# yalue/cudabrot

Measured on AMD Instinct MI355X. Metric: Msamples/sec (escaping points) + HBM GB/s, 4096x4096 max_iter=20000, 1/2/4/8 GPU, higher is better.
Workload: dtype f64

## Files before the change

### cudabrot_amd/capi.py

```python

import ctypes as C
import os

import numpy as np

CB_DEFAULT_THREADS = 512 * 512
CB_SAMPLES_PER_THREAD = 50
CB_DEFAULT_RNG_SEED = 1337
CB_KERNEL_DEFAULT = 0
CB_KERNEL_SIMPLE = 1
CB_KERNEL_TIMED = 2
CB_KERNEL_FULL_ITERATE = 3
CB_TONE_AUTO, CB_TONE_LUT, CB_TONE_THRESHOLDS = 0, 1, 2
CB_KERNEL_FLAG_BURNING_SHIP = 0x100
CB_KERNEL_FLAG_DRAIN = 0x200
CB_KERNEL_FLAG_ANTI = 0x400
CB_POWER_MIN, CB_POWER_MAX = 3, 8
CB_KERNEL_POWER_MASK = 0xF000


def CB_KERNEL_POWER(degree):
    degree = int(degree)
    if not CB_POWER_MIN <= degree <= CB_POWER_MAX:
        raise ValueError("degree must be an integer from %d to %d" % (CB_POWER_MIN, CB_POWER_MAX))
# ... 82 lines not shown
            "cycles_replay",
            "cycles_total",
            "rt_not_first_start",
            "rt_last_end",
            "rt_wave_life_sum",
        )
    ]

    def as_dict(self):
        return {n: int(getattr(self, n)) for n, _ in self._fields_}


class ScatterArray(C.Structure):

    _fields_ = [("offset", C.c_uint64), ("bytes", C.c_uint64)]


SCATTER_ARRAYS = ("wave_count stream a_count a_base grouped region_start region_count region_group owner_first "
                  "group_first group_regions n_regions chunk_desc chunk_list run_start slice_base sorted").split()


class ScatterLayout(C.Structure):

    _fields_ = [
        (n, C.c_uint32)
        for n in ("enabled n_waves cap n_tiles tiles_x tiles_y n_planes two_level n_groups chunked chunks_per_wave "
                  "max_regions e_row_shift e_col_mask e_row_mask e_chan_shift e_chan_mask reserved").split()
    ] + [(n, ScatterArray) for n in SCATTER_ARRAYS]

    def arrays(self):
        return {n: (int(getattr(self, n).offset), int(getattr(self, n).bytes))
                for n in SCATTER_ARRAYS if getattr(self, n).bytes}


def _share_torch_hip_runtime():
    if os.environ.get("CUDABROT_AMD_SYSTEM_HIP") == "1":
        return None
    try:
        import importlib.util

        spec = importlib.util.find_spec("torch")
    except (ImportError, ValueError):
        spec = None
    if spec is None or not spec.submodule_search_locations:
        return None
    cand = os.path.join(list(spec.submodule_search_locations)[0], "lib", "libamdhip64.so")
    if not os.path.exists(cand):
        return None
    C.CDLL(cand, mode=C.RTLD_GLOBAL)
    return cand


def _load():
    path = library_path()
    if not os.path.exists(path):
        raise ImportError(
            "cudabrot_amd: %s is missing -- build it with `make` (or __graft_entry__.build()); "
            "there is no CPU fallback" % path
        )
    _share_torch_hip_runtime()
    lib_ = C.CDLL(path)
    vp, u32, u64, i32 = C.c_void_p, C.c_uint32, C.c_uint64, C.c_int
    dims_p, it_p, cnt_p = C.POINTER(FractalDimensions), C.POINTER(IterationControl), C.POINTER(Counters)
    col_p = C.POINTER(ColorParams)
    sigs = {
        "cb_abi_version": (i32, []),
        "cb_error_string": (C.c_char_p, [i32]),
        "cb_debug_knob": (C.c_char_p, [C.c_char_p]),
        "cb_debug_last_draw_kernel": (i32, []),
        "cb_debug_interior_map_level": (i32, []),
        "cb_renderer_interior_map_level": (i32, [vp]),
        "cb_recompute_pixel_deltas": (i32, [dims_p, C.POINTER(C.c_char_p)]),
        "cb_rng_state_bytes": (C.c_size_t, [u32]),
        "cb_initialize_rng": (i32, [u64, u64, u32, vp, vp]),
        "cb_scatter_workspace_bytes": (C.c_size_t, [dims_p, u32, u32]),
        "cb_scatter_workspace_bytes_channels": (C.c_size_t, [dims_p, i32, u32, u32]),
        "cb_draw_buddhabrot": (i32, [dims_p, vp, it_p, vp, u32, u32, vp, i32, vp, C.c_size_t, vp, vp]),
        "cb_carry_bytes": (C.c_size_t, [u32]),
        "cb_draw_buddhabrot_channels": (i32, [dims_p, vp, it_p, i32, vp, u32, u32, vp, i32, vp, C.c_size_t, vp, vp]),
        "cb_flush_scatter_channels": (i32, [dims_p, vp, i32, u32, vp, C.c_size_t, vp]),
        "cb_renderer_finish": (i32, [vp]),
        "cb_flush_scatter": (i32, [dims_p, vp, u32, vp, C.c_size_t, vp]),
        "cb_debug_scatter_layout": (i32, [dims_p, i32, u32, vp, C.c_size_t, C.POINTER(ScatterLayout)]),
        "cb_renderer_create": (i32, [C.POINTER(vp), i32, dims_p, it_p, u64, u64, u32]),
        "cb_renderer_create_channels": (i32, [C.POINTER(vp), i32, dims_p, it_p, i32, u64, u64, u32]),
        "cb_renderer_grayscale_plane": (i32, [vp, i32, C.c_double, i32, vp, C.POINTER(u64), C.POINTER(C.c_double)]),
        "cb_renderer_render_passes": (i32, [vp, u32, i32]),
        "cb_renderer_prepare": (i32, [vp, i32]),
        "cb_renderer_read_histogram": (i32, [vp, vp]),
        "cb_renderer_write_histogram": (i32, [vp, vp]),
        "cb_renderer_read_counters": (i32, [vp, cnt_p]),
        "cb_renderer_read_rng_states": (i32, [vp, vp]),
        "cb_renderer_write_rng_states": (i32, [vp, vp]),
        "cb_renderer_device_histogram": (vp, [vp]),
        "cb_renderers_reduce": (i32, [C.POINTER(vp), i32]),
        "cb_renderer_destroy": (None, [vp]),
        "cb_set_grayscale_pixels": (None, [vp, i32, i32, C.c_double, vp, C.POINTER(u64), C.POINTER(C.c_double)]),
        "cb_save_image": (i32, [C.c_char_p, vp, i32, i32]),
        "cb_save_image_be": (i32, [C.c_char_p, vp, i32, i32]),
        "cb_tone_value": (C.c_uint16, [u64, u64, C.c_double]),
        "cb_tone_map_device": (i32, [vp, i32, i32, C.c_double, i32, vp, C.POINTER(u64), C.POINTER(C.c_double), vp]),
        "cb_renderer_grayscale_image": (i32, [vp, C.c_double, i32, vp, C.POINTER(u64), C.POINTER(C.c_double)]),
        "cb_compose_color": (i32, [C.POINTER(vp), i32, i32, col_p, vp, vp]),
        "cb_compose_color_device": (i32, [C.POINTER(vp), i32, i32, C.c_double, i32, col_p, vp, vp, vp]),
        "cb_renderer_color_image": (i32, [vp, C.POINTER(i32), C.c_double, i32, col_p, vp, vp]),
        "cb_save_ppm_be": (i32, [C.c_char_p, vp, i32, i32]),
        "cb_focus_mask_bytes": (C.c_size_t, [i32]),
        "cb_focus_probe": (i32, [dims_p, it_p, vp, u32, u32, i32, vp, vp, i32, vp]),
        "cb_focus_cells": (i32, [i32, vp, i32, vp, C.POINTER(u32)]),
        "cb_draw_buddhabrot_focus": (i32, [dims_p, vp, it_p, vp, u32, u32, vp, i32, i32, vp, u32, vp]),
        "cb_renderer_set_focus": (i32, [vp, i32, u32, i32, i32]),
        "cb_renderer_focus_cells": (i32, [vp, C.POINTER(u32), C.POINTER(u32)]),
        "cb_draw_buddhabrot_projected": (i32, [dims_p, vp, it_p, C.POINTER(C.c_double), vp, u32, u32, vp, i32, vp]),
        "cb_renderer_set_projection": (i32, [vp, C.POINTER(C.c_double)]),
        "cb_renderer_projection": (i32, [vp, C.POINTER(C.c_double)]),
    }
    for name, (res, args) in sigs.items():
        fn = getattr(lib_, name)
        fn.restype = res
        fn.argtypes = args
    return lib_


lib = _load()
EXPORTED_SYMBOLS = (
    "cb_abi_version cb_error_string cb_debug_knob cb_debug_last_draw_kernel cb_debug_interior_map_level cb_renderer_interior_map_level cb_recompute_pixel_deltas cb_rng_state_bytes cb_initialize_rng "
    "cb_scatter_workspace_bytes cb_scatter_workspace_bytes_channels cb_carry_bytes cb_draw_buddhabrot cb_flush_scatter cb_renderer_create "
    "cb_renderer_render_passes cb_renderer_finish "
    "cb_renderer_read_histogram "
    "cb_renderer_write_histogram cb_renderer_read_counters cb_renderer_device_histogram "
    "cb_renderer_destroy cb_set_grayscale_pixels cb_save_image cb_save_image_be cb_tone_value "
    "cb_tone_map_device cb_renderer_grayscale_image cb_renderer_read_rng_states cb_renderer_write_rng_states "
    "cb_draw_buddhabrot_channels cb_flush_scatter_channels cb_renderer_create_channels cb_renderer_grayscale_plane cb_renderers_reduce "
    "cb_renderer_prepare cb_compose_color cb_compose_color_device cb_renderer_color_image cb_save_ppm_be "
    "cb_focus_mask_bytes cb_focus_probe cb_focus_cells cb_draw_buddhabrot_focus cb_renderer_set_focus cb_renderer_focus_cells "
    "cb_draw_buddhabrot_projected cb_renderer_set_projection cb_renderer_projection cb_debug_scatter_layout"
).split()


def _error_string(code):
    return lib.cb_error_string(int(code)).decode()


def _check(code, what):
    if code != 0:
        raise CudabrotError(code, what)


def recompute_pixel_deltas(dims):
    msg = C.c_char_p()
    ok = lib.cb_recompute_pixel_deltas(C.byref(dims), C.byref(msg))
    return bool(ok), (None if ok else msg.value.decode())


def rng_state_bytes(n_threads):
    return int(lib.cb_rng_state_bytes(n_threads))


def initialize_rng(seed, first_subsequence, n_threads, d_states, stream=0):
    _check(lib.cb_initialize_rng(seed, first_subsequence, n_threads, d_states, stream), "cb_initialize_rng")


def scatter_workspace_bytes(dims, n_threads, samples_per_thread, n_channels=1):
    return int(lib.cb_scatter_workspace_bytes_channels(C.byref(dims), n_channels, n_threads, samples_per_thread))


def carry_bytes(n_threads):
    return int(lib.cb_carry_bytes(n_threads))


def draw_buddhabrot(dims, d_hist, iterations, d_states, n_threads, samples_per_thread, d_counters=0,
                    kernel_variant=CB_KERNEL_DEFAULT, stream=0, d_workspace=0, workspace_bytes=0, d_carry=0):
    _check(
        lib.cb_draw_buddhabrot(C.byref(dims), d_hist, C.byref(iterations), d_states, n_threads,
                               samples_per_thread, d_counters, kernel_variant, d_workspace, workspace_bytes,
                               d_carry, stream),
        "cb_draw_buddhabrot",
    )


def flush_scatter(dims, d_hist, n_threads, d_workspace, workspace_bytes, stream=0):
    _check(lib.cb_flush_scatter(C.byref(dims), d_hist, n_threads, d_workspace, workspace_bytes, stream),
           "cb_flush_scatter")


def debug_scatter_layout(dims, n_threads, d_workspace, workspace_bytes, n_channels=0):
    out = ScatterLayout()
    _check(lib.cb_debug_scatter_layout(C.byref(dims), n_channels, n_threads, d_workspace, workspace_bytes,
                                       C.byref(out)), "cb_debug_scatter_layout")
    return out


def focus_mask_bytes(level):
    return int(lib.cb_focus_mask_bytes(int(level)))


def focus_probe(dims, iterations, d_states, n_threads, samples_per_thread, level, d_mask, d_counters=0,
                kernel_variant=CB_KERNEL_DEFAULT, stream=0):
    _check(
        lib.cb_focus_probe(C.byref(dims), C.byref(iterations), d_states, n_threads, samples_per_thread, int(level),
                           d_mask, d_counters, kernel_variant, stream),
        "cb_focus_probe",
    )


def focus_cells(level, mask, dilate=1):
    m = np.ascontiguousarray(mask, dtype=np.uint32).reshape(-1)
    if m.size * 4 != focus_mask_bytes(level):
        raise ValueError("mask size does not match the level")
    n = C.c_uint32()
    _check(lib.cb_focus_cells(int(level), m.ctypes.data, int(dilate), None, C.byref(n)), "cb_focus_cells")
    cells = np.empty(int(n.value), dtype=np.uint32)
    _check(lib.cb_focus_cells(int(level), m.ctypes.data, int(dilate), cells.ctypes.data, C.byref(n)), "cb_focus_cells")
    return cells


def draw_buddhabrot_focus(dims, d_hist, iterations, d_states, n_threads, samples_per_thread, d_counters=0,
                          kernel_variant=CB_KERNEL_DEFAULT, level=0, d_cells=0, n_cells=0, stream=0):
    _check(
# ... 237 lines not shown
```

### cudabrot_amd/csrc/scatter.hip

```cpp
#include <stdlib.h>
#include <string.h>

#include <type_traits>

#include "kernels.h"

namespace cb {

namespace {

constexpr int kSortPrioIo = 3;
constexpr int kSortPrioRank = 0;
constexpr int kGatherPrio = 0;
constexpr uint32_t kLeanBatch = 4;

constexpr uint32_t kScatterThreads = 512;
constexpr uint32_t kChunkEntries = 8192;
constexpr uint32_t kPerThread = kChunkEntries / kScatterThreads;
constexpr uint32_t kAccThreadsWide = 1024;
constexpr uint32_t kGroupShift = 10;
static_assert((1u << kGroupShift) == kGroupTiles, "group = tile >> kGroupShift");
constexpr uint32_t kReplicas = kGroupReplicas;
constexpr uint32_t kMaxGroups = 256;
constexpr uint32_t kMaxKeys = kMaxGroups * kGroupTiles;
// ... 93 lines not shown
  const uint32_t n_owners = owner_count(b);
  const uint32_t per = (n_owners + 1023u) / 1024u;
  const uint32_t o0 = threadIdx.x * per;
  if (threadIdx.x == 0) all_entries = 0ull;
  __syncthreads();
  uint32_t mine = 0;
  unsigned long long my_entries = 0;
  for (uint32_t k = 0; k < per; ++k) {
    if (o0 + k < n_owners) {
      unsigned long long begin, entries;
      uint32_t piece;
      owner_extent(b, o0 + k, &begin, &entries, &piece);
      mine += (uint32_t) ((entries + piece - 1u) / piece);
      my_entries += entries;
    }
  }
  if (my_entries) __hip_atomic_fetch_add(&all_entries, my_entries, __ATOMIC_RELAXED, __HIP_MEMORY_SCOPE_WORKGROUP);
  uint32_t total = 0;
  uint32_t r = block_exclusive_scan(mine, wave_totals, &total);
  if (threadIdx.x == 0) {
    *reinterpret_cast<unsigned long long *>(b.n_regions + 2) = b.chunked ? all_entries * kChunkWords : all_entries;
  }
  for (uint32_t k = 0; k < per; ++k) {
    const uint32_t o = o0 + k;
    if (o >= n_owners) break;
    unsigned long long begin, entries;
    uint32_t piece;
    owner_extent(b, o, &begin, &entries, &piece);
    const uint32_t regions = (uint32_t) ((entries + piece - 1u) / piece);
    b.owner_first[o] = r;
    if (b.two_level) {
      b.group_first[o] = r;
      b.group_regions[o] = regions;
    }
    r += regions;
  }
  if (threadIdx.x == 0) {
    b.owner_first[n_owners] = total;
    *b.n_regions = total;
    if (!b.two_level) {
      b.group_first[0] = 0u;
      b.group_regions[0] = total;
    }
  }
}

__global__ void __launch_bounds__(256) bin_fill_regions_kernel(BinLayout b) {
  const uint32_t r = blockIdx.x * blockDim.x + threadIdx.x;
  if (r >= *b.n_regions) return;
  uint32_t lo = 0, hi = owner_count(b);
  while (hi - lo > 1u) {
    const uint32_t mid = (lo + hi) >> 1;
    if (b.owner_first[mid] <= r) {
      lo = mid;
    } else {
      hi = mid;
    }
  }
  unsigned long long begin, entries;
  uint32_t piece;
  owner_extent(b, lo, &begin, &entries, &piece);
  const unsigned long long offset = (unsigned long long) (r - b.owner_first[lo]) * piece;
  b.region_start[r] = begin + offset;
  b.region_count[r] = (uint32_t) ((entries - offset) < piece ? (entries - offset) : piece);
  b.region_group[r] = b.two_level ? lo : 0u;
}

constexpr uint32_t kSliceTargetGroups = 12288;
constexpr uint32_t kSliceTargetGroupsTwoLevel = 6144;
static_assert(kSliceTargetGroupsTwoLevel <= kSliceTargetGroups, "the grid of the gather is sized by the larger one");
constexpr uint32_t kSliceRegionsMin = 512;
constexpr uint32_t kSliceEntriesMin = 32768;
__device__ __forceinline__ uint32_t slice_regions_for(const BinLayout &b, unsigned long long pairs,
                                                      unsigned long long entries) {
  const unsigned long long target = b.two_level ? kSliceTargetGroupsTwoLevel : kSliceTargetGroups;
  unsigned long long s = (pairs + target - 1u) / target;
  if (s < kSliceRegionsMin) s = kSliceRegionsMin;
  const unsigned long long by_entries = entries ? (kSliceEntriesMin * pairs + entries - 1u) / entries : b.slice_regions;
  if (s < by_entries) s = by_entries;
  if (s > b.slice_regions) s = b.slice_regions;
  return (uint32_t) s;
}

__global__ void __launch_bounds__(1024) bin_slice_table_kernel(BinLayout b) {
  __shared__ uint32_t wave_totals[16];
  const uint32_t nk = b.n_tiles;
  const uint32_t per = (nk + 1023u) / 1024u;
  const uint32_t t0 = threadIdx.x * per;
  unsigned long long pairs = 0;
  for (uint32_t g = 0; g < b.n_groups; ++g) {
    const uint32_t tiles = (nk - (g << kGroupShift)) < kGroupTiles ? (nk - (g << kGroupShift)) : kGroupTiles;
    pairs += (unsigned long long) tiles * b.group_regions[g];
  }
  const uint32_t S = slice_regions_for(b, pairs, *reinterpret_cast<const unsigned long long *>(b.n_regions + 2));
  if (threadIdx.x == 0) b.n_regions[1] = S;
  auto slices_of = [&](uint32_t t) { return (b.group_regions[t >> kGroupShift] + S - 1u) / S; };
  uint32_t mine = 0;
  for (uint32_t k = 0; k < per; ++k) {
    if (t0 + k < nk) mine += slices_of(t0 + k);
  }
  uint32_t total = 0;
  uint32_t run = block_exclusive_scan(mine, wave_totals, &total);
  for (uint32_t k = 0; k < per; ++k) {
    const uint32_t t = t0 + k;
    if (t < nk) {
      b.slice_base[t] = run;
      run += slices_of(t);
    }
  }
  if (threadIdx.x == 0) b.slice_base[nk] = total;
}

constexpr uint32_t kDummyPlace = kRegionEntries + 8u;
template <bool kFewTiles>
struct SortLds {
  static constexpr uint32_t kReplicas = kFewTiles ? 8u : 2u;
  static constexpr uint32_t kStride = (kFewTiles ? 256u : kGroupTiles) + 16u;
  static constexpr size_t kBytes =
      (kReplicas * kStride + 16 + 2 * kRegionChunks + 4) * sizeof(uint32_t) + (kRegionEntries + 16) * sizeof(uint16_t);
};
constexpr uint32_t kFewTilesMax = 256;
constexpr uint32_t kSortGrid = 32768;
constexpr uint32_t kRunBatch = 8;

template <bool kPlain>
__device__ __forceinline__ uint32_t sort_word(uint32_t e, uint32_t k0, const BinLayout &b) {
  if (kPlain) {
    const uint32_t key = __umul24(e >> (16 + kTileShift), b.tiles_x) + ((e & 0xffffu) >> kTileShift) - k0;
    return (key << 16) | ((e >> (16 - kTileShift)) & ((kTileSize - 1u) << kTileShift)) | (e & (kTileSize - 1u));
  }
  return ((tile_of(e, b) - k0) << 16) | offset_of(e, b);
}

template <bool kPlain, bool kFewTiles, bool kChunked = false, bool kLean = false>
__global__ void __launch_bounds__(kSortThreads, 8) bin_region_sort_kernel(BinLayout b, uint32_t skip_lean) {
  constexpr uint32_t kCntReplicas = SortLds<kFewTiles>::kReplicas, kCntStride = SortLds<kFewTiles>::kStride;
  constexpr uint32_t kDummyKey = kCntStride - 16u;
  __builtin_amdgcn_s_setprio(kSortPrioIo);
  extern __shared__ uint32_t lds[];
  uint32_t *cnt = lds + (threadIdx.x % kCntReplicas) * kCntStride;
  uint32_t *wave_totals = lds + kCntReplicas * kCntStride;
  uint2 *chunks = reinterpret_cast<uint2 *>(lds + kCntReplicas * kCntStride + 16);
  uint16_t *image = reinterpret_cast<uint16_t *>(lds + kCntReplicas * kCntStride + 16 + 2 * kRegionChunks + 4);

  const uint32_t n_regions = *b.n_regions;
  constexpr uint32_t kBatchRegions = kLean ? kRunBatch : 1u;
  for (uint32_t r_batch = blockIdx.x * kBatchRegions; r_batch < n_regions; r_batch += gridDim.x * kBatchRegions) {
  uint32_t runs[4] = {0u, 0u, 0u, 0u};
  const auto push_run = [&](uint32_t v) {
    runs[0] = __builtin_amdgcn_alignbit(runs[1], runs[0], 16);
    runs[1] = __builtin_amdgcn_alignbit(runs[2], runs[1], 16);
    runs[2] = __builtin_amdgcn_alignbit(runs[3], runs[2], 16);
    runs[3] = __builtin_amdgcn_alignbit(v, runs[3], 16);
  };
#pragma unroll 1
  for (uint32_t r = r_batch; r < r_batch + kBatchRegions; ++r) {
  if (kLean && r >= n_regions) {
    push_run(0u);
    continue;
  }
  uint32_t n = kChunked ? 0u : b.region_count[r];
  const unsigned long long start = kChunked ? (unsigned long long) r * kRegionEntries : b.region_start[r];
  const uint32_t *src = kChunked ? b.stream : (b.two_level ? b.grouped : b.stream) + start;
  const uint32_t k0 = b.region_group[r] << kGroupShift;
  const uint32_t nk = (b.n_tiles - k0) < kGroupTiles ? (b.n_tiles - k0) : kGroupTiles;
  __syncthreads();
  for (uint32_t t = threadIdx.x; t < kCntReplicas * kCntStride; t += kSortThreads) lds[t] = 0u;
  if (kChunked && threadIdx.x < 64u) {
    const uint32_t n_chunks = b.region_count[r];
    const uint2 c = threadIdx.x < n_chunks && threadIdx.x < kRegionChunks ? b.chunk_list[b.region_start[r] + threadIdx.x]
                                                                          : make_uint2(0u, 0u);
    if (threadIdx.x < kRegionChunks) chunks[threadIdx.x] = c;
    uint32_t words = c.y;
#pragma unroll
    for (uint32_t d = 32; d >= 1; d >>= 1) words += __shfl_xor(words, d, 64);
    if (threadIdx.x == 0) chunks[kRegionChunks].x = words;
  }
  __syncthreads();
  if (kChunked) n = chunks[kRegionChunks].x;

  const bool lean_region = kPlain && n != 0u && (kChunked || (start & 7ull) == 0ull);
  if (!kLean && skip_lean != 0u && lean_region) continue;
  if (kLean && !lean_region) {
    push_run(0u);
    continue;
  }
  if constexpr (kLean) {
    typedef __attribute__((address_space(3))) uint32_t *LdsWord;
    typedef __attribute__((address_space(3))) uint16_t *LdsHalf;
    const uint32_t lds0 = (uint32_t) reinterpret_cast<uintptr_t>(static_cast<void *>(lds));
    const uint32_t cnt_at = lds0 + (uint32_t) ((threadIdx.x % kCntReplicas) * kCntStride * sizeof(uint32_t)) - (k0 << 2);
    const uint32_t image_at = (uint32_t) reinterpret_cast<uintptr_t>(static_cast<void *>(image));
    const uint4 *src4 = reinterpret_cast<const uint4 *>(src);
// ... 150 lines not shown
        const uint32_t i4 = (half * (kSortPerThread / 8u) + j) * kSortThreads + threadIdx.x;
        v[j] = src4[i4 < last4 ? i4 : last4];
      }
#pragma unroll
      for (uint32_t j = 0; j < kSortPerThread / 8u; ++j) {
        asm volatile("" : "+v"(v[j].x), "+v"(v[j].y), "+v"(v[j].z), "+v"(v[j].w));
        const uint32_t k = half * (kSortPerThread / 8u) + j;
        const uint32_t i = (k * kSortThreads + threadIdx.x) * 4u;
        const uint32_t w0 = sort_word<kPlain>(v[j].x, k0, b), w1 = sort_word<kPlain>(v[j].y, k0, b);
        const uint32_t w2 = sort_word<kPlain>(v[j].z, k0, b), w3 = sort_word<kPlain>(v[j].w, k0, b);
        e[4 * k + 0] = (i >= head && i < lim) ? w0 : ~0u;
        e[4 * k + 1] = (i + 1u >= head && i + 1u < lim) ? w1 : ~0u;
        e[4 * k + 2] = (i + 2u >= head && i + 2u < lim) ? w2 : ~0u;
        e[4 * k + 3] = (i + 3u < lim) ? w3 : ~0u;
      }
#pragma unroll
      for (uint32_t k = half * (kSortPerThread / 2u); k < (half + 1u) * (kSortPerThread / 2u); ++k) {
        const uint32_t key = e[k] >> 16;
        lds_inc(&cnt[key < kDummyKey ? key : kDummyKey]);
      }
    }
  }
  __syncthreads();
  __builtin_amdgcn_s_setprio(kSortPrioRank);
  {
    const bool has_key = threadIdx.x < kDummyKey;
    uint32_t c[kCntReplicas], sum = 0;
#pragma unroll
    for (uint32_t k = 0; k < kCntReplicas; ++k) {
      c[k] = has_key ? lds[k * kCntStride + threadIdx.x] : 0u;
      sum += c[k];
    }
    uint32_t first = sort_exclusive_scan(sum, wave_totals);
    __syncthreads();
    if (threadIdx.x < nk) b.run_start[(size_t) threadIdx.x * b.max_regions + r] = (uint16_t) first;
#pragma unroll
    for (uint32_t k = 0; k < kCntReplicas; ++k) {
      if (has_key) lds[k * kCntStride + threadIdx.x] = first;
      first += c[k];
    }
  }
  __syncthreads();
  const uint32_t shift = (uint32_t) (start & 7ull);
#pragma unroll
  for (uint32_t k = 0; k < kSortPerThread; ++k) {
    const uint32_t key = e[k] >> 16;
    const bool real = key < kDummyKey;
    const uint32_t pos = __hip_atomic_fetch_add(&cnt[real ? key : kDummyKey], 1u, __ATOMIC_RELAXED,
                                                __HIP_MEMORY_SCOPE_WORKGROUP);
    image[real ? shift + pos : kDummyPlace] = (uint16_t) e[k];
  }
  __syncthreads();
  __builtin_amdgcn_s_setprio(kSortPrioIo);
  uint16_t *dst = b.sorted + (start - shift);
  const uint32_t lo = shift, hi = shift + n;
  const uint32_t body_lo = (lo + 7u) & ~7u, body_hi = hi & ~7u;
  if (body_lo < body_hi) {
    for (uint32_t i = lo + threadIdx.x; i < body_lo; i += kSortThreads) dst[i] = image[i];
    const uint4 *s4 = reinterpret_cast<const uint4 *>(image);
    uint4 *d4 = reinterpret_cast<uint4 *>(dst);
    for (uint32_t i = (body_lo >> 3) + threadIdx.x; i < (body_hi >> 3); i += kSortThreads) d4[i] = s4[i];
    for (uint32_t i = body_hi + threadIdx.x; i < hi; i += kSortThreads) dst[i] = image[i];
  } else {
    for (uint32_t i = lo + threadIdx.x; i < hi; i += kSortThreads) dst[i] = image[i];
  }
  if (kChunked && threadIdx.x == 0) b.region_count[r] = n;
  }
  }
  if (kLean && threadIdx.x < (b.n_tiles < kGroupTiles ? b.n_tiles : kGroupTiles)) {
    *reinterpret_cast<uint4 *>(b.run_start + (size_t) threadIdx.x * b.max_regions + r_batch) =
        make_uint4(runs[0], runs[1], runs[2], runs[3]);
  }
  }
}


template <uint32_t kAccThreads, bool kMaskedAdds>
__global__ void __launch_bounds__(kAccThreads) bin_gather_accumulate_kernel(BinLayout b,
                                                                            unsigned long long *hist,
                                                                            int w, int h) {
  __shared__ uint32_t tile[kTilePixels];
  __builtin_amdgcn_s_setprio(kGatherPrio);
  const uint32_t s = blockIdx.x;
  if (s >= b.slice_base[b.n_tiles]) return;
  uint32_t lo = 0, hi = b.n_tiles;
  while (hi - lo > 1u) {
    const uint32_t mid = (lo + hi) >> 1;
    if (b.slice_base[mid] <= s) {
      lo = mid;
    } else {
      hi = mid;
    }
  }
  const uint32_t t = lo;
  const uint32_t g = t >> kGroupShift, kl = t & (kGroupTiles - 1u);
  const uint32_t k0 = g << kGroupShift;
  const uint32_t nk = (b.n_tiles - k0) < kGroupTiles ? (b.n_tiles - k0) : kGroupTiles;
  const uint32_t first = b.group_first[g], n_reg = b.group_regions[g];
  const uint32_t S = b.n_regions[1];
  const uint32_t r0 = (s - b.slice_base[t]) * S;
  const uint32_t r1 = (r0 + S < n_reg) ? r0 + S : n_reg;

  for (uint32_t p = threadIdx.x; p < (uint32_t) kTilePixels; p += kAccThreads) tile[p] = 0u;
  __syncthreads();
  const uint16_t *row0 = b.run_start + (size_t) kl * b.max_regions + first;
  const bool last_key = (kl + 1u == nk);
  const uint16_t *row1 = row0 + b.max_regions;
  const uint32_t lane = threadIdx.x & 63u, wv = threadIdx.x >> 6;
  struct Run {
    const uint4 *p4;
    uint32_t lead, len;
  };
  const auto describe = [&](uint32_t base) -> Run {
    Run run = {reinterpret_cast<const uint4 *>(b.sorted), 0u, 0u};
    const uint32_t rr = base + lane;
    if (rr < r1) {
      const unsigned long long rs = b.chunked ? (unsigned long long) (first + rr) * kRegionEntries : b.region_start[first + rr];
      const unsigned long long beg = rs + row0[rr];
      const unsigned long long end = rs + (last_key ? b.region_count[first + rr] : (uint32_t) row1[rr]);
      if (end != beg) {
        run.lead = (uint32_t) (beg & 7ull);
        run.len = run.lead + (uint32_t) (end - beg);
        run.p4 = reinterpret_cast<const uint4 *>(b.sorted + (beg - run.lead));
      }
    }
    return run;
  };
  constexpr uint32_t kStep = (kAccThreads / 64u) * 64u;
  Run next = describe(r0 + wv * 64u);
  for (uint32_t base = r0 + wv * 64u; base < r1; base += kStep) {
    const Run run = next;
    next = describe(base + kStep);
    const uint32_t lead = run.lead, len = run.len;
    const uint4 *p4 = run.p4;
    const uint32_t last8 = len ? (len - 1u) >> 3 : 0u;
    for (uint32_t at = 0; __ballot(at < len) != 0ull; at += 32u) {
      if (at < len) {
        uint4 v[4];
#pragma unroll
        for (uint32_t j = 0; j < 4; ++j) {
          const uint32_t i8 = (at >> 3) + j;
          v[j] = p4[i8 < last8 ? i8 : last8];
        }
#pragma unroll
        for (uint32_t j = 0; j < 4; ++j) {
          const uint32_t i0 = at + 8u * j;
          if (__ballot(i0 < len) == 0ull) break;
          const uint32_t words[4] = {v[j].x, v[j].y, v[j].z, v[j].w};
          if (__ballot(i0 < lead || i0 + 8u > len) == 0ull) {
#pragma unroll
            for (uint32_t q = 0; q < 8; ++q) lds_inc(&tile[(words[q >> 1] >> ((q & 1u) * 16u)) & 0xffffu]);
            continue;
          }
          if constexpr (kMaskedAdds) {
            const int lo = (int) lead - (int) i0, hi = (int) len - (int) i0;
            const uint32_t lo_c = (uint32_t) (lo < 0 ? 0 : (lo > 8 ? 8 : lo)), hi_c = (uint32_t) (hi < 0 ? 0 : (hi > 8 ? 8 : hi));
            const uint32_t valid = hi_c > lo_c ? ((1u << (hi_c - lo_c)) - 1u) << lo_c : 0u;
#pragma unroll
            for (uint32_t q = 0; q < 8; ++q) {
              __hip_atomic_fetch_add(&tile[(words[q >> 1] >> ((q & 1u) * 16u)) & 0xffffu], (valid >> q) & 1u,
                                     __ATOMIC_RELAXED, __HIP_MEMORY_SCOPE_WORKGROUP);
            }
          } else {
#pragma unroll
            for (uint32_t q = 0; q < 8; ++q) {
              const uint32_t i = i0 + q;
              if (i >= lead && i < len) lds_inc(&tile[(words[q >> 1] >> ((q & 1u) * 16u)) & 0xffffu]);
            }
          }
        }
      }
    }
  }
  __syncthreads();
  const uint32_t plane_tiles = b.tiles_x * b.tiles_y;
  const uint32_t plane = t / plane_tiles, tt = t - plane * plane_tiles;
  const uint32_t row_0 = (tt / b.tiles_x) << kTileShift;
  const uint32_t col_0 = (tt % b.tiles_x) << kTileShift;
  hist += (unsigned long long) plane * b.plane_pixels;
  for (uint32_t p = threadIdx.x; p < (uint32_t) kTilePixels; p += kAccThreads) {
    const uint32_t v = tile[p];
    if (v != 0u) {
      const uint32_t row = row_0 + (p >> kTileShift);
// ... 354 lines not shown
    b.a_count = carve<uint32_t>(p, keys * n_waves * sizeof(uint32_t), sizes.a_count);
    b.a_base = carve<unsigned long long>(p, (keys + 1) * sizeof(unsigned long long), sizes.a_base);
  }
  b.stream = carve<uint32_t>(p, (size_t) n_waves * b.cap * sizeof(uint32_t), sizes.stream);
  if (b.chunked) {
    b.chunk_desc = carve<uint32_t>(p, (size_t) n_waves * b.chunks_per_wave * sizeof(uint32_t), sizes.chunk_desc);
    b.chunk_list = carve<uint2>(p, (size_t) n_waves * b.chunks_per_wave * sizeof(uint2), sizes.chunk_list);
    b.sorted = carve<uint16_t>(p, (size_t) b.max_regions * kRegionEntries * sizeof(uint16_t), sizes.sorted);
  } else {
    if (b.two_level) b.grouped = carve<uint32_t>(p, (size_t) n_waves * b.cap * sizeof(uint32_t), sizes.grouped);
    b.sorted = carve<uint16_t>(p, (size_t) n_waves * b.cap * sizeof(uint16_t), sizes.sorted);
  }
  b.enabled = 1;
  if (carved) *carved = sizes;
  return b;
}

constexpr uint32_t kChainDelayUs = 40;
__global__ void __launch_bounds__(64) chain_delay_kernel(uint32_t ticks) {
  const unsigned long long t0 = wall_clock64();
  for (uint32_t turn = 0; turn < 4096u && wall_clock64() - t0 < ticks; ++turn) __builtin_amdgcn_s_sleep(32);
}

hipError_t launch_binned_scatter(const BinLayout &b, unsigned long long *hist, int w, int h,
                                 hipStream_t stream) {
  if (!b.enabled) return hipSuccess;
  hipLaunchKernelGGL(chain_delay_kernel, dim3(1), dim3(64), 0, stream, kChainDelayUs * 100u);
  if (b.chunked) {
    hipLaunchKernelGGL(chunk_count_kernel, dim3(b.n_waves), dim3(64), 0, stream, b);
    hipLaunchKernelGGL(group_scan_rows_kernel, dim3(b.n_groups), dim3(256), 0, stream, b);
    hipLaunchKernelGGL(group_scan_keys_kernel, dim3(1), dim3(1024), 0, stream, b);
    hipLaunchKernelGGL(chunk_list_kernel, dim3(b.n_waves), dim3(64), 0, stream, b);
  } else if (b.two_level) {
    const uint32_t nk = b.n_groups * kReplicas;
    hipLaunchKernelGGL(group_count_kernel, dim3(b.n_waves), dim3(kScatterThreads), nk * sizeof(uint32_t), stream, b);
    hipLaunchKernelGGL(group_scan_rows_kernel, dim3(nk), dim3(256), 0, stream, b);
    hipLaunchKernelGGL(group_scan_keys_kernel, dim3(1), dim3(1024), 0, stream, b);
    const size_t scatter_lds = ((size_t) 3 * nk + 8 + 2 * kChunkEntries) * sizeof(uint32_t);
    if (scatter_lds > 64 * 1024) {
      hipError_t e = hipFuncSetAttribute(reinterpret_cast<const void *>(group_scatter_kernel),
                                         hipFuncAttributeMaxDynamicSharedMemorySize, (int) scatter_lds);
      if (e != hipSuccess) return e;
    }
    hipLaunchKernelGGL(group_scatter_kernel, dim3(b.n_waves), dim3(kScatterThreads), scatter_lds, stream, b);
  }
  hipLaunchKernelGGL(bin_region_heads_kernel, dim3(1), dim3(1024), 0, stream, b);
  hipLaunchKernelGGL(bin_fill_regions_kernel, dim3((b.max_regions + 255u) / 256u), dim3(256), 0, stream, b);
  hipLaunchKernelGGL(bin_slice_table_kernel, dim3(1), dim3(1024), 0, stream, b);
  const bool plain = b.n_planes == 1u && b.e_row_shift == 16u && b.e_col_mask == 0xffffu && b.e_row_mask == 0xffffu &&
                     b.e_chan_mask == 0u;
  const bool few = b.n_tiles <= kFewTilesMax;
  uint32_t skip_lean = 0u;
  const auto launch_sort = [&](auto kernel, size_t lds_bytes, uint32_t batch = 1u) -> hipError_t {
    const hipError_t e = hipFuncSetAttribute(reinterpret_cast<const void *>(kernel),
                                             hipFuncAttributeMaxDynamicSharedMemorySize, (int) lds_bytes);
    if (e != hipSuccess) return e;
    const uint32_t batches = (b.max_regions + batch - 1u) / batch;
    const uint32_t grid = batches < kSortGrid ? batches : kSortGrid;
    hipLaunchKernelGGL(kernel, dim3(grid), dim3(kSortThreads), lds_bytes, stream, b, skip_lean);
    return hipSuccess;
  };
  hipError_t se;
  if (b.chunked) {
    se = plain ? launch_sort(bin_region_sort_kernel<true, false, true, true>, SortLds<false>::kBytes, kRunBatch)
               : launch_sort(bin_region_sort_kernel<false, false, true>, SortLds<false>::kBytes);
  } else if (plain && !b.two_level && b.tiles_x <= 128u) {
    se = few ? launch_sort(bin_region_sort_kernel<true, true, false, true>, SortLds<true>::kBytes, kRunBatch)
             : launch_sort(bin_region_sort_kernel<true, false, false, true>, SortLds<false>::kBytes, kRunBatch);
    if (se == hipSuccess && (b.cap & 7u) != 0u) {
      skip_lean = 1u;
      se = few ? launch_sort(bin_region_sort_kernel<true, true>, SortLds<true>::kBytes)
               : launch_sort(bin_region_sort_kernel<true, false>, SortLds<false>::kBytes);
    }
  } else if (few) {
    se = plain ? launch_sort(bin_region_sort_kernel<true, true>, SortLds<true>::kBytes)
               : launch_sort(bin_region_sort_kernel<false, true>, SortLds<true>::kBytes);
  } else {
    se = plain ? launch_sort(bin_region_sort_kernel<true, false>, SortLds<false>::kBytes)
               : launch_sort(bin_region_sort_kernel<false, false>, SortLds<false>::kBytes);
  }
  if (se != hipSuccess) return se;
  const unsigned long long rows = b.n_tiles < kGroupTiles ? b.n_tiles : kGroupTiles;
  const unsigned long long by_cap = rows * b.max_regions / b.slice_regions;
  const unsigned long long slices = b.n_tiles + (by_cap > kSliceTargetGroups ? by_cap : kSliceTargetGroups) + 1ull;
  const auto launch_gather = [&](auto kernel) {
    hipLaunchKernelGGL(kernel, dim3((uint32_t) slices), dim3(kAccThreadsWide), 0, stream, b, hist, w, h);
  };
  if (b.two_level) launch_gather(bin_gather_accumulate_kernel<kAccThreadsWide, true>);
  else launch_gather(bin_gather_accumulate_kernel<kAccThreadsWide, false>);
  return hipGetLastError();
}

}
```

### include/cudabrot_amd.h

```cpp
#ifndef CUDABROT_AMD_H_
#define CUDABROT_AMD_H_

#include <stddef.h>
#include <stdint.h>

#ifdef __cplusplus
extern "C" {
#endif

#define CB_ABI_VERSION 1

#define CB_DEFAULT_BLOCK_SIZE 512
#define CB_DEFAULT_BLOCK_COUNT 512
#define CB_DEFAULT_THREADS (CB_DEFAULT_BLOCK_SIZE * CB_DEFAULT_BLOCK_COUNT)
#define CB_SAMPLES_PER_THREAD 50
#define CB_DEFAULT_RNG_SEED 1337ull

typedef uint64_t cb_pixel;

typedef struct {
  int w;
  int h;
  double min_real;
  double min_imag;
// ... 98 lines not shown
                                 int kernel_variant, void *stream);


typedef struct cb_renderer cb_renderer;

int cb_renderer_create(cb_renderer **out, int device, const cb_fractal_dimensions *dims,
                       const cb_iteration_control *iterations, uint64_t seed,
                       uint64_t first_subsequence, uint32_t n_threads);
int cb_renderer_create_channels(cb_renderer **out, int device, const cb_fractal_dimensions *dims,
                                const cb_iteration_control *windows, int n_channels, uint64_t seed,
                                uint64_t first_subsequence, uint32_t n_threads);
int cb_renderer_render_passes(cb_renderer *r, uint32_t passes, int kernel_variant);
int cb_renderer_set_focus(cb_renderer *r, int level, uint32_t probe_passes, int dilate, int kernel_variant);
int cb_renderer_focus_cells(const cb_renderer *r, uint32_t *n_cells, uint32_t *n_total);
int cb_renderer_set_projection(cb_renderer *r, const double projection[8]);
int cb_renderer_projection(const cb_renderer *r, double out[8]);
int cb_renderer_prepare(cb_renderer *r, int kernel_variant);
int cb_renderer_finish(cb_renderer *r);
int cb_renderer_read_histogram(cb_renderer *r, cb_pixel *host_out);
int cb_renderer_write_histogram(cb_renderer *r, const cb_pixel *host_in);
int cb_renderer_read_counters(cb_renderer *r, cb_counters *host_out);
int cb_renderer_read_rng_states(cb_renderer *r, void *host_out);
int cb_renderer_write_rng_states(cb_renderer *r, const void *host_in);
cb_pixel *cb_renderer_device_histogram(cb_renderer *r);
int cb_renderers_reduce(cb_renderer *const *renderers, int n);
void cb_renderer_destroy(cb_renderer *r);


void cb_set_grayscale_pixels(const cb_pixel *hist, int w, int h, double gamma, uint16_t *gray_out,
                             uint64_t *max_out, double *scale_out);
int cb_save_image(const char *path, uint16_t *gray, int w, int h);

uint16_t cb_tone_value(uint64_t count, uint64_t max, double gamma);
int cb_save_image_be(const char *path, const uint16_t *gray_be, int w, int h);


#define CB_TONE_AUTO 0
#define CB_TONE_LUT 1
#define CB_TONE_THRESHOLDS 2

int cb_tone_map_device(const cb_pixel *d_hist, int w, int h, double gamma, int mode,
                       uint16_t *d_gray_be, uint64_t *max_out, double *scale_out, void *stream);
int cb_renderer_grayscale_image(cb_renderer *r, double gamma, int mode, uint16_t *host_gray_be,
                                uint64_t *max_out, double *scale_out);

int cb_renderer_grayscale_plane(cb_renderer *r, int plane, double gamma, int mode, uint16_t *host_gray_be,
                                uint64_t *max_out, double *scale_out);

#define CB_COMPOSE_RGB 0
#define CB_COMPOSE_HSL 1
typedef struct {
  int compose;
  double black_percent;
  double white_percent;
  double hue_shift;
} cb_color_params;

int cb_compose_color(const uint16_t *const gray[3], int w, int h, const cb_color_params *p, uint16_t *rgb_be,
                     uint16_t levels[6]);
int cb_compose_color_device(const cb_pixel *const d_hist[3], int w, int h, double gamma, int tone_mode,
                            const cb_color_params *p, uint16_t *d_rgb_be, uint16_t levels[6], void *stream);
int cb_renderer_color_image(cb_renderer *r, const int planes[3], double gamma, int tone_mode,
                            const cb_color_params *p, uint16_t *host_rgb_be, uint16_t levels[6]);
int cb_save_ppm_be(const char *path, const uint16_t *rgb_be, int w, int h);

const char *cb_error_string(int code);
int cb_abi_version(void);

const char *cb_debug_knob(const char *name);
typedef struct cb_scatter_array {
  uint64_t offset;
  uint64_t bytes;
} cb_scatter_array;
typedef struct cb_scatter_layout {
  uint32_t enabled, n_waves, cap, n_tiles, tiles_x, tiles_y, n_planes, two_level, n_groups, chunked, chunks_per_wave,
      max_regions;
  uint32_t e_row_shift, e_col_mask, e_row_mask, e_chan_shift, e_chan_mask;
  uint32_t reserved;
  cb_scatter_array wave_count, stream, a_count, a_base, grouped, region_start, region_count, region_group, owner_first,
      group_first, group_regions, n_regions, chunk_desc, chunk_list, run_start, slice_base, sorted;
} cb_scatter_layout;
int cb_debug_scatter_layout(const cb_fractal_dimensions *dims, int n_channels, uint32_t n_threads,
                            const void *d_workspace, size_t workspace_bytes, cb_scatter_layout *out);
int cb_debug_last_draw_kernel(void);
int cb_debug_interior_map_level(void);
int cb_renderer_interior_map_level(const cb_renderer *r);

#ifdef __cplusplus
}
#endif
#endif
```

Baseline: 119,500.

## Reorder gather blocks so adjacent tiles share region slices across XCDs

```diff
diff --git a/cudabrot_amd/capi.py b/cudabrot_amd/capi.py
--- a/cudabrot_amd/capi.py
+++ b/cudabrot_amd/capi.py
@@ -188,6 +188,7 @@
         "cb_renderer_finish": (i32, [vp]),
         "cb_flush_scatter": (i32, [dims_p, vp, u32, vp, C.c_size_t, vp]),
         "cb_debug_scatter_layout": (i32, [dims_p, i32, u32, vp, C.c_size_t, C.POINTER(ScatterLayout)]),
+        "cb_debug_gather_order": (u32, [u32, u32, u32, C.POINTER(u32), C.POINTER(u32)]),
         "cb_renderer_create": (i32, [C.POINTER(vp), i32, dims_p, it_p, u64, u64, u32]),
         "cb_renderer_create_channels": (i32, [C.POINTER(vp), i32, dims_p, it_p, i32, u64, u64, u32]),
         "cb_renderer_grayscale_plane": (i32, [vp, i32, C.c_double, i32, vp, C.POINTER(u64), C.POINTER(C.c_double)]),
@@ -240,7 +241,7 @@
     "cb_draw_buddhabrot_channels cb_flush_scatter_channels cb_renderer_create_channels cb_renderer_grayscale_plane cb_renderers_reduce "
     "cb_renderer_prepare cb_compose_color cb_compose_color_device cb_renderer_color_image cb_save_ppm_be "
     "cb_focus_mask_bytes cb_focus_probe cb_focus_cells cb_draw_buddhabrot_focus cb_renderer_set_focus cb_renderer_focus_cells "
-    "cb_draw_buddhabrot_projected cb_renderer_set_projection cb_renderer_projection cb_debug_scatter_layout"
+    "cb_draw_buddhabrot_projected cb_renderer_set_projection cb_renderer_projection cb_debug_scatter_layout cb_debug_gather_order"
 ).split()
 
 
diff --git a/cudabrot_amd/csrc/scatter.hip b/cudabrot_amd/csrc/scatter.hip
--- a/cudabrot_amd/csrc/scatter.hip
+++ b/cudabrot_amd/csrc/scatter.hip
@@ -199,11 +199,25 @@
   return (uint32_t) s;
 }
 
+constexpr uint32_t kXcds = 8;
+constexpr uint32_t kGatherGroupTiles = 2;
+__host__ __device__ inline uint32_t gather_order_size(uint32_t n_tiles, uint32_t n_slices) {
+  const uint32_t units = (n_tiles + kGatherGroupTiles - 1u) / kGatherGroupTiles * n_slices;
+  return (units + kXcds - 1u) / kXcds * kXcds * kGatherGroupTiles;
+}
+__host__ __device__ inline bool gather_order(uint32_t i, uint32_t n_tiles, uint32_t n_slices, uint32_t *tile,
+                                             uint32_t *slice) {
+  const uint32_t place = i / kXcds;
+  const uint32_t u = place / kGatherGroupTiles * kXcds + i % kXcds;
+  const uint32_t units_per_slice = (n_tiles + kGatherGroupTiles - 1u) / kGatherGroupTiles;
+  *slice = u / units_per_slice;
+  *tile = (u % units_per_slice) * kGatherGroupTiles + place % kGatherGroupTiles;
+  return *slice < n_slices && *tile < n_tiles;
+}
+
 __global__ void __launch_bounds__(1024) bin_slice_table_kernel(BinLayout b) {
   __shared__ uint32_t wave_totals[16];
   const uint32_t nk = b.n_tiles;
-  const uint32_t per = (nk + 1023u) / 1024u;
-  const uint32_t t0 = threadIdx.x * per;
   unsigned long long pairs = 0;
   for (uint32_t g = 0; g < b.n_groups; ++g) {
     const uint32_t tiles = (nk - (g << kGroupShift)) < kGroupTiles ? (nk - (g << kGroupShift)) : kGroupTiles;
@@ -211,21 +225,16 @@
   }
   const uint32_t S = slice_regions_for(b, pairs, *reinterpret_cast<const unsigned long long *>(b.n_regions + 2));
   if (threadIdx.x == 0) b.n_regions[1] = S;
-  auto slices_of = [&](uint32_t t) { return (b.group_regions[t >> kGroupShift] + S - 1u) / S; };
+  static_assert(kMaxGroups <= 1024, "a thread per group");
   uint32_t mine = 0;
-  for (uint32_t k = 0; k < per; ++k) {
-    if (t0 + k < nk) mine += slices_of(t0 + k);
+  if (threadIdx.x < b.n_groups) {
+    const uint32_t k0 = threadIdx.x << kGroupShift;
+    mine = gather_order_size((nk - k0) < kGroupTiles ? (nk - k0) : kGroupTiles, (b.group_regions[threadIdx.x] + S - 1u) / S);
   }
   uint32_t total = 0;
-  uint32_t run = block_exclusive_scan(mine, wave_totals, &total);
-  for (uint32_t k = 0; k < per; ++k) {
-    const uint32_t t = t0 + k;
-    if (t < nk) {
-      b.slice_base[t] = run;
-      run += slices_of(t);
-    }
-  }
-  if (threadIdx.x == 0) b.slice_base[nk] = total;
+  const uint32_t before = block_exclusive_scan(mine, wave_totals, &total);
+  if (threadIdx.x < b.n_groups) b.slice_base[threadIdx.x] = before;
+  if (threadIdx.x == 0) b.slice_base[b.n_groups] = total;
 }
 
 constexpr uint32_t kDummyPlace = kRegionEntries + 8u;
@@ -542,8 +551,8 @@
   __shared__ uint32_t tile[kTilePixels];
   __builtin_amdgcn_s_setprio(kGatherPrio);
   const uint32_t s = blockIdx.x;
-  if (s >= b.slice_base[b.n_tiles]) return;
-  uint32_t lo = 0, hi = b.n_tiles;
+  if (s >= b.slice_base[b.n_groups]) return;
+  uint32_t lo = 0, hi = b.n_groups;
   while (hi - lo > 1u) {
     const uint32_t mid = (lo + hi) >> 1;
     if (b.slice_base[mid] <= s) {
@@ -552,13 +561,15 @@
       hi = mid;
     }
   }
-  const uint32_t t = lo;
-  const uint32_t g = t >> kGroupShift, kl = t & (kGroupTiles - 1u);
+  const uint32_t g = lo;
   const uint32_t k0 = g << kGroupShift;
   const uint32_t nk = (b.n_tiles - k0) < kGroupTiles ? (b.n_tiles - k0) : kGroupTiles;
   const uint32_t first = b.group_first[g], n_reg = b.group_regions[g];
   const uint32_t S = b.n_regions[1];
-  const uint32_t r0 = (s - b.slice_base[t]) * S;
+  uint32_t kl, slice;
+  if (!gather_order(s - b.slice_base[g], nk, (n_reg + S - 1u) / S, &kl, &slice)) return;
+  const uint32_t t = k0 + kl;
+  const uint32_t r0 = slice * S;
   const uint32_t r1 = (r0 + S < n_reg) ? r0 + S : n_reg;
 
   for (uint32_t p = threadIdx.x; p < (uint32_t) kTilePixels; p += kAccThreads) tile[p] = 0u;
@@ -1079,7 +1090,10 @@
   if (se != hipSuccess) return se;
   const unsigned long long rows = b.n_tiles < kGroupTiles ? b.n_tiles : kGroupTiles;
   const unsigned long long by_cap = rows * b.max_regions / b.slice_regions;
-  const unsigned long long slices = b.n_tiles + (by_cap > kSliceTargetGroups ? by_cap : kSliceTargetGroups) + 1ull;
+  const unsigned long long smallest = b.slice_regions < kSliceRegionsMin ? b.slice_regions : kSliceRegionsMin;
+  const unsigned long long empty = (kGatherGroupTiles - 1ull) * (b.max_regions / smallest + b.n_groups) +
+                                   (unsigned long long) (kXcds - 1u) * kGatherGroupTiles * b.n_groups;
+  const unsigned long long slices = b.n_tiles + (by_cap > kSliceTargetGroups ? by_cap : kSliceTargetGroups) + 1ull + empty;
   const auto launch_gather = [&](auto kernel) {
     hipLaunchKernelGGL(kernel, dim3((uint32_t) slices), dim3(kAccThreadsWide), 0, stream, b, hist, w, h);
   };
@@ -1089,3 +1103,12 @@
 }
 
 }
+
+extern "C" uint32_t cb_debug_gather_order(uint32_t n_tiles, uint32_t n_slices, uint32_t count, uint32_t *tiles,
+                                          uint32_t *slices) {
+  const uint32_t size = cb::gather_order_size(n_tiles, n_slices);
+  for (uint32_t i = 0; i < count && i < size && tiles && slices; ++i) {
+    if (!cb::gather_order(i, n_tiles, n_slices, &tiles[i], &slices[i])) tiles[i] = slices[i] = 0xffffffffu;
+  }
+  return size;
+}
diff --git a/include/cudabrot_amd.h b/include/cudabrot_amd.h
--- a/include/cudabrot_amd.h
+++ b/include/cudabrot_amd.h
@@ -204,6 +204,7 @@
 } cb_scatter_layout;
 int cb_debug_scatter_layout(const cb_fractal_dimensions *dims, int n_channels, uint32_t n_threads,
                             const void *d_workspace, size_t workspace_bytes, cb_scatter_layout *out);
+uint32_t cb_debug_gather_order(uint32_t n_tiles, uint32_t n_slices, uint32_t count, uint32_t *tiles, uint32_t *slices);
 int cb_debug_last_draw_kernel(void);
 int cb_debug_interior_map_level(void);
 int cb_renderer_interior_map_level(const cb_renderer *r);
```

After: 94820. 0.793x the previous value.
